# junyanz/interactive-deep-colorization

Hardware: NVIDIA B200
Metric: net_forward images/sec @256x256 (higher is better)
Workload: dtype f16x2-split operands, f32 accumulate (ab within 1e-3 of the f32 reference)

## Files before the change

### interactive_deep_colorization_b200/csrc/idc_api.cu

```cuda
#include <math.h>
#include <stdarg.h>
#include <stdio.h>
#include <string.h>

#include <algorithm>

#include "idc_internal.h"

using namespace idc;

struct idc_ctx : public idc::Ctx {};

namespace {

int fail(Ctx* c, int code, const char* fmt, ...) {
  char buf[512];
  va_list ap;
  va_start(ap, fmt);
  vsnprintf(buf, sizeof(buf), fmt, ap);
  va_end(ap);
  if (c) c->err = buf;
  return code;
}

// ... 616 lines not shown
  c->simt = flags & IDC_FLAG_ENGINE_SIMT;
  c->fast = (flags & IDC_FLAG_FAST_FP16) && !c->simt;
  c->dist = flags & IDC_FLAG_DIST;
  c->glob = flags & IDC_FLAG_GLOBAL_HINTS;
  c->caffe313 = flags & IDC_FLAG_CAFFE313;
  build_plan(c);
  int rc = alloc_workspace(c);
  if (rc != IDC_OK) {
    fprintf(stderr, "idc_create: %s\n", c->err.c_str());
    idc_destroy(c);
    return rc;
  }
  cudaStreamCreateWithFlags(&c->own_stream, cudaStreamNonBlocking);
  *out = c;
  return IDC_OK;
}

int idc_set_option(idc_ctx* c, const char* name, int value) {
  if (!c || !name) return IDC_ERR_ARG;
  struct { const char* n; int* v; } tab[] = {
      {"halo", &c->opt.halo}, {"pairs", &c->opt.pairs}, {"mt", &c->opt.mt}, {"chunk_kb", &c->opt.chunk_kb},
      {"split_k", &c->opt.split_k}, {"direct_stores", &c->opt.direct_stores}, {"host_pipe", &c->opt.host_pipe},
      {"pdl", &c->opt.pdl}, {"split_pairs", &c->opt.split_pairs}, {"tanh_scale", &c->opt.tanh_scale},
      {"side_dist", &c->opt.side_dist}, {"split_bn128", &c->opt.split_bn128}, {"halo_split", &c->opt.halo_split}, {"prologue_sync2", &c->opt.prologue_sync2}, {"chain", &c->opt.chain}, {"conv1_1_umma", &c->opt.conv1_1_umma}};
  for (auto& t : tab)
    if (!strcmp(t.n, name)) {
      *t.v = value;
      if (c->weights_ready && strcmp(name, "host_pipe") && strcmp(name, "tanh_scale") && strcmp(name, "side_dist") && strcmp(name, "conv1_1_umma")) {
        CUDA_TRY(c, cudaSetDevice(c->dev));
        CUDA_TRY(c, cudaDeviceSynchronize());
        int rc = plan_engines(c);
        if (rc != IDC_OK) return rc;
      }
      if (c->graph_exec) { cudaGraphExecDestroy(c->graph_exec); c->graph_exec = nullptr; }
      return IDC_OK;
    }
  return fail(c, IDC_ERR_KEY, "unknown option '%s'", name);
}

int idc_load_tensor(idc_ctx* c, const char* key, const void* data, int dtype, int ndim, const int64_t* dims) {
  if (!c || !key || !data || ndim < 0 || ndim > 8 || (ndim && !dims)) return fail(c, IDC_ERR_ARG, "bad load_tensor args");
  HostTensor t;
  size_t count = 1;
  for (int i = 0; i < ndim; ++i) {
    if (dims[i] < 0) return fail(c, IDC_ERR_ARG, "negative dim");
    t.dims.push_back(dims[i]);
    count *= (size_t)dims[i];
// ... 728 lines not shown
```

### interactive_deep_colorization_b200/csrc/idc_internal.h

```cpp
#pragma once
#include <cuda.h>
#include <cuda_fp16.h>
#include <cuda_runtime.h>
#include <stdint.h>

#include <map>
#include <string>
#include <vector>

#include "../../include/idc_b200.h"

namespace idc {

constexpr int kMaxTaps = 34;
constexpr int kMaxSrc = 6;
constexpr int kMaxCls = 4;

enum Act { ACT_NONE = 0, ACT_RELU = 1, ACT_LEAKY02 = 2 };

constexpr int kActScaleLog2 = 6;
constexpr float kActScale = 64.0f;
constexpr float kActInvScale = 1.0f / 64.0f;

struct Tap {
// ... 55 lines not shown
  double flops_per_image = 0;
};

struct Conv11Weights {
  float w[36 * 64];
  float b[64];
};

struct Options {
  int halo = 1;
  int pairs = 1;
  int mt = -1;
  int chunk_kb = -1;
  int split_k = -1;
  int direct_stores = 0;
  int host_pipe = 1;
  int pdl = 1;
  int split_pairs = 1;
  int split_bn128 = 1;
  int conv1_1_umma = 1;
  int chain = 0;
  int prologue_sync2 = 1;
  int halo_split = 0;
  int side_dist = 1;
  int tanh_scale = 110;
};

struct HostTensor {
  std::vector<float> data;
  std::vector<int64_t> dims;
};

struct Ctx {
  int dev = 0;
  int max_n = 0, H = 0, W = 0;
  unsigned flags = 0;
  Options opt;
  bool simt = false, fast = false, dist = false, glob = false;
  std::map<std::string, HostTensor> raw;
  std::vector<ActBuf> bufs;
  std::map<std::string, int> buf_index;
  std::vector<ConvOp> ops;
  char* arena = nullptr;
  size_t arena_bytes = 0;
  bool weights_ready = false;
  float* w11 = nullptr;
// ... 122 lines not shown
```

### interactive_deep_colorization_b200/csrc/idc_umma.cu

```cuda
#include <stdio.h>
#include <stdlib.h>

#include "idc_internal.h"

#ifndef IDC_CTA_COUNTERS
#define IDC_CTA_COUNTERS 0
#endif

namespace idc {

constexpr int kBM = 128;
constexpr int kBK = 64;
constexpr int kThreads = 384;
constexpr int kCtrlRegs = 56;
constexpr int kAccRegs = 224;
constexpr int kAccThreads = 256;

struct UmmaParams {
  const CUtensorMap* amaps;
  const int4* kblk;
  int nkb, ncls;
  int chunk_kb;
  int split_k;
  float* ws;
// ... 2 lines not shown
  int hbox, wbox, wshift;
  int Hl, Wl, cout_pad;
  const float* bias;
  const float* scale;
  const float* shift;
  const float* gadd;
  int gadd_ld;
  float gadd_mult;
  int act;
  __half* out_hi;
  __half* out_lo;
  int Hout, Wout, Cout, os;
  int store_mode;
  float* out_f32;
  int out_ld;
  const float* wout;
  const float* bout;
  float* out_ab;
  float out_mult;
  int* err;
  long long* dbgbuf;
  int n_amaps;
  int max_ctas;
  int halo_groups;
  int prologue_sync2;
  int img0;
};

__device__ __forceinline__ uint32_t smem_u32(const void* p) { return (uint32_t)__cvta_generic_to_shared(p); }

__device__ __forceinline__ void mbar_init(uint32_t bar, uint32_t count) {
  asm volatile("mbarrier.init.shared::cta.b64 [%0], %1;" ::"r"(bar), "r"(count));
}
__device__ __forceinline__ void mbar_expect_tx(uint32_t bar, uint32_t bytes) {
  asm volatile("mbarrier.arrive.expect_tx.shared::cta.b64 _, [%0], %1;" ::"r"(bar), "r"(bytes) : "memory");
}
__device__ __forceinline__ void mbar_arrive(uint32_t bar) {
  asm volatile("mbarrier.arrive.shared::cta.b64 _, [%0];" ::"r"(bar) : "memory");
}
__device__ __forceinline__ uint32_t mbar_try_wait(uint32_t bar, uint32_t parity) {
  uint32_t ok;
  asm volatile(
      "{\n\t.reg .pred p;\n\t"
      "mbarrier.try_wait.parity.shared::cta.b64 p, [%1], %2;\n\t"
      "selp.u32 %0, 1, 0, p;\n\t}"
      : "=r"(ok)
      : "r"(bar), "r"(parity)
// ... 168 lines not shown
  return r;
}

template <bool SPLIT>
__device__ __forceinline__ void split_pack(const float (&f)[32], uint32_t (&hw)[16], uint32_t (&lw)[16]) {
#pragma unroll
  for (int j = 0; j < 16; ++j) {
    hw[j] = pack_f16x2_sat(f[2 * j], f[2 * j + 1]);
    if (SPLIT) {
      const float2 hf = __half22float2(*reinterpret_cast<const __half2*>(&hw[j]));
      lw[j] = pack_f16x2_sat(f[2 * j] - hf.x, f[2 * j + 1] - hf.y);
    }
  }
}

__device__ __forceinline__ void split_h(float v, __half& hi, __half& lo) {
  v = fminf(fmaxf(v, -65504.f), 65504.f);
  hi = __float2half_rn(v);
  lo = __float2half_rn(v - __half2float(hi));
}

constexpr int kHaloW = 10, kHaloH = 18;
constexpr int kHaloPlane = (kHaloW * kHaloH * 128 + 1023) / 1024 * 1024;
template <int BN, int MT, int CG, bool SPLIT, bool HALO = false>
struct SmemPlan {
  static constexpr int kABytes = MT * kBM * kBK * 2;
  static constexpr int kAStage = HALO ? 0 : kABytes;
  static constexpr int kBBytes = (BN / CG) * kBK * 2;
  static constexpr int kStageBytes = (SPLIT ? 2 : 1) * (kAStage + kBBytes);
  static constexpr int kHaloSlot = (SPLIT ? 2 : 1) * kHaloPlane;
  static constexpr int kHaloBytes = HALO ? 2 * kHaloSlot : 0;
  static_assert(!HALO || MT == 1, "halo tiles are single 16x8-pixel M-tiles");
  static constexpr int kTail = 3 * BN * 4 + 272 * 4 + 256 + 128 * 2 * 4;
  static constexpr int kOutStage = 16384;
  static constexpr int kBudget = 232448 - 1024 - kTail - kOutStage - kHaloBytes;
  static constexpr int kStages = kBudget / kStageBytes >= 4 ? 4 : kBudget / kStageBytes;
  static constexpr int kTotal = kStages * kStageBytes + kHaloBytes + kOutStage + kTail + 1024;
  static constexpr int kBufCols = MT * BN;
  static constexpr int kNBuf = (512 / kBufCols) >= 4 ? 4 : (512 / kBufCols);
  static constexpr int kTmemCols = (kNBuf * kBufCols <= 128) ? 128 : (kNBuf * kBufCols <= 256 ? 256 : 512);
  static constexpr int kCH = (MT == 2) ? BN : BN / 2;
  static_assert(kStages >= 2, "need at least a double-buffered operand ring");
  static_assert(CG == 1 || BN == 256 || BN == 128 || BN == 64, "pairs: BN/2 weight rows per CTA must be a whole number of swizzle atoms");
};

template <int BN, int MT, int CG, bool SPLIT, bool HALO, bool CHAIN>
__device__ __forceinline__ void conv_body(const CUtensorMap* bhi_list, const CUtensorMap* blo_list,
                                          const UmmaParams* plist, const int nl, int* gridbar) {
  static_assert(!(HALO && CHAIN), "chained launches use per-tap boxes");
  using SP = SmemPlan<BN, MT, CG, SPLIT, HALO>;
  const UmmaParams& p0 = plist[0];
  constexpr int STAGES = SP::kStages;
  constexpr bool PAIR = CG == 2;
  extern __shared__ uint8_t smem_raw[];
  uint8_t* smem = reinterpret_cast<uint8_t*>((reinterpret_cast<uintptr_t>(smem_raw) + 1023) & ~uintptr_t(1023));
  uint8_t* s_halo = smem + STAGES * SP::kStageBytes;
  uint8_t* s_out = s_halo + SP::kHaloBytes;
  uint8_t* tail = s_out + SP::kOutStage;
  float* s_bias = reinterpret_cast<float*>(tail);
  float* s_scale = s_bias + BN;
  float* s_shift = s_scale + BN;
  float* s_head = s_shift + BN;
  uint64_t* s_bar = reinterpret_cast<uint64_t*>(s_head + 272);
  constexpr int NBUF = SP::kNBuf;
  uint64_t* full_bar = s_bar;
  uint64_t* empty_bar = s_bar + STAGES;
  uint64_t* tfull_bar = s_bar + 2 * STAGES;
  uint64_t* tempty_bar = s_bar + 2 * STAGES + NBUF;
  uint32_t* s_tmem = reinterpret_cast<uint32_t*>(s_bar + 2 * STAGES + 2 * NBUF);
  uint64_t* afull_bar = s_bar + 20;
  uint64_t* aempty_bar = s_bar + 22;
  float* s_red = reinterpret_cast<float*>(s_bar + 32);

  const int warp = threadIdx.x >> 5, lane = threadIdx.x & 31;
  const long long t_kernel0 = (IDC_CTA_COUNTERS && p0.dbgbuf) ? clock64() : 0;

  if (!CHAIN && p0.wout) {
    for (int i = threadIdx.x; i < 256; i += kThreads) s_head[i] = p0.wout[i];
    if (threadIdx.x < 2) s_head[256 + threadIdx.x] = p0.bout[threadIdx.x];
  }
  const uint32_t cta_rank = PAIR ? cluster_ctarank() : 0u;
  const bool leader = cta_rank == 0;
  if (threadIdx.x == 32) {
    prefetch_tmap(bhi_list);
    if (SPLIT) prefetch_tmap(blo_list);
    for (int i = 0; i < p0.n_amaps; ++i) prefetch_tmap(p0.amaps + i);
  }
  if (threadIdx.x == 0) {
    for (int s = 0; s < STAGES; ++s) {
      mbar_init(smem_u32(&full_bar[s]), CG);
      mbar_init(smem_u32(&empty_bar[s]), 1);
    }
    for (int a = 0; a < NBUF; ++a) {
      mbar_init(smem_u32(&tfull_bar[a]), 1);
      mbar_init(smem_u32(&tempty_bar[a]), 8 * CG);
    }
    if (HALO)
      for (int a = 0; a < 2; ++a) {
        mbar_init(smem_u32(&afull_bar[a]), CG);
        mbar_init(smem_u32(&aempty_bar[a]), 1);
      }
    asm volatile("fence.mbarrier_init.release.cluster;" ::: "memory");
  }
  if (PAIR && p0.prologue_sync2) cluster_sync_all();
  if (warp == 1) {
    if (PAIR) {
      asm volatile("tcgen05.alloc.cta_group::2.sync.aligned.shared::cta.b32 [%0], %1;" ::"r"(smem_u32(s_tmem)),
                   "r"((uint32_t)SP::kTmemCols)
                   : "memory");
      asm volatile("tcgen05.relinquish_alloc_permit.cta_group::2.sync.aligned;" ::: "memory");
    } else {
      asm volatile("tcgen05.alloc.cta_group::1.sync.aligned.shared::cta.b32 [%0], %1;" ::"r"(smem_u32(s_tmem)),
                   "r"((uint32_t)SP::kTmemCols)
                   : "memory");
      asm volatile("tcgen05.relinquish_alloc_permit.cta_group::1.sync.aligned;" ::: "memory");
    }
  }
  tc_fence_before();
  if (PAIR) cluster_sync_all(); else __syncthreads();
  tc_fence_after();
  const uint32_t tmem_base = *s_tmem;
// ... 58 lines not shown
        pdl_wait();
      } else if (w0 < p.total_tiles * S) {
        grid_wait(gridbar, l * (int)gridDim.x, p.err);
        asm volatile("fence.proxy.async;" ::: "memory");
      }
      for (int w = w0; w < p.total_tiles * S; w += gridDim.x / CG) {
        const int tile = w / S, ks = w - tile * S;
        const int kbeg = (ks * p.nkb) / S, kend = ((ks + 1) * p.nkb) / S;
        const int kpre = (w == w0) ? kbeg + npre : kbeg;
        int r = tile;
        const int nt = r % p.n_tiles_n;
        r /= p.n_tiles_n;
        const int cls = r % p.ncls;
        r /= p.ncls;
        if (PAIR) r = 2 * r + (int)cta_rank;
        const int img_rel = r / tiles_per_img;
        r -= img_rel * tiles_per_img;
        const int img = p.img0 + img_rel;
        const int y0 = (r / p.tiles_x) * (p.hbox * MT), x0 = (r % p.tiles_x) * p.wbox;
        const int brow = cls * p.cout_pad + nt * BN + (int)cta_rank * (BN / CG);
        const int4* kb = p.kblk + cls * p.nkb;
        if (HALO) {
          for (int k = kbeg; k < kend; ++k) {
            if (k % 9 == 0) {
              const uint32_t slot = hcount & 1, hphase = (hcount >> 1) & 1;
              ++hcount;
              mbar_wait(smem_u32(&aempty_bar[slot]), hphase ^ 1, p.err, 6);
              if (elect_one()) {
                const uint32_t fa = smem_u32(&afull_bar[slot]);
                const uint32_t sh = smem_u32(s_halo + slot * SP::kHaloSlot);
                const int c0 = (k / 9) * kBK;
                constexpr uint32_t kHaloTx = (SPLIT ? 2 : 1) * kHaloW * kHaloH * 128;
                if (PAIR) {
                  if (leader) mbar_expect_tx(fa, 2 * kHaloTx); else mbar_arrive_rank0(fa);
                  tma_load_4d_pair(sh, p.amaps, fa, c0, x0 - 1, y0 - 1, img);
                  if (SPLIT) tma_load_4d_pair(sh + kHaloPlane, p.amaps + 1, fa, c0, x0 - 1, y0 - 1, img);
                } else {
                  mbar_expect_tx(fa, kHaloTx);
                  tma_load_4d(sh, p.amaps, fa, c0, x0 - 1, y0 - 1, img);
                  if (SPLIT) tma_load_4d(sh + kHaloPlane, p.amaps + 1, fa, c0, x0 - 1, y0 - 1, img);
                }
              }
              __syncwarp();
            }
            mbar_wait(smem_u32(&empty_bar[stage]), phase ^ 1, p.err, 1);
            if (k >= kpre && elect_one()) {
              const uint32_t fb = smem_u32(&full_bar[stage]);
              const int4 e = __ldg(kb + k);
              const uint32_t sb = smem_u32(smem + stage * SP::kStageBytes);
              if (PAIR) {
                if (leader) mbar_expect_tx(fb, 2 * SP::kStageBytes); else mbar_arrive_rank0(fb);
                tma_load_2d_pair(sb, &bmap_hi, fb, e.y, brow);
                if (SPLIT) tma_load_2d_pair(sb + SP::kBBytes, &bmap_lo, fb, e.y, brow);
              } else {
                mbar_expect_tx(fb, SP::kStageBytes);
                tma_load_2d(sb, &bmap_hi, fb, e.y, brow);
                if (SPLIT) tma_load_2d(sb + SP::kBBytes, &bmap_lo, fb, e.y, brow);
              }
            }
            __syncwarp();
            if (++stage == STAGES) { stage = 0; phase ^= 1; }
          }
        }
        if (!HALO)
        for (int k = kbeg; k < kend; ++k) {
          mbar_wait(smem_u32(&empty_bar[stage]), phase ^ 1, p.err, 1);
          if (elect_one()) {
            const uint32_t fb = smem_u32(&full_bar[stage]);
            const int4 e = __ldg(kb + k);
            const uint32_t sa = smem_u32(smem + stage * SP::kStageBytes);
            const CUtensorMap* am = p.amaps + e.x;
// ... 19 lines not shown
          }
          __syncwarp();
          if (++stage == STAGES) { stage = 0; phase ^= 1; }
        }
      }
      }
    }
  } else if (warp == 1 && leader) {
    {
      constexpr uint32_t idesc = make_idesc(BN, kBM * CG);
      int stage = 0;
      uint32_t phase = 0;
      uint32_t cc = 0;
      uint32_t hcount = 0;
      long long t_wait_tempty = 0, t_wait_full = 0, t_first_full = 0;
      const long long t_start = clock64();
      for (int l = 0; l < n_layers; ++l) {
      const UmmaParams& p = plist[l];
      const int G = p.chunk_kb;
      const int S = p.split_k;
      for (int w = blockIdx.x / CG; w < p.total_tiles * S; w += gridDim.x / CG) {
        const int ks = w % S;
        const int kbeg = (ks * p.nkb) / S, kend = ((ks + 1) * p.nkb) / S;
        for (int k0 = kbeg; k0 < kend; k0 += G, ++cc) {
          const uint32_t buf = cc % NBUF;
          const uint32_t bphase = (cc / NBUF) & 1;
          const long long tA = (IDC_CTA_COUNTERS && p.dbgbuf) ? clock64() : 0;
          mbar_wait(smem_u32(&tempty_bar[buf]), bphase ^ 1, p.err, 2);
          if (IDC_CTA_COUNTERS && p.dbgbuf) t_wait_tempty += clock64() - tA;
          tc_fence_after();
          const uint32_t d_tmem = tmem_base + buf * SP::kBufCols;
          const int k1 = (k0 + G < kend) ? k0 + G : kend;
          for (int k = k0; k < k1; ++k) {
            const long long tB = (IDC_CTA_COUNTERS && p.dbgbuf) ? clock64() : 0;
            uint32_t hslot = 0;
            if (HALO) {
              if (k % 9 == 0) {
                mbar_wait(smem_u32(&afull_bar[hcount & 1]), (hcount >> 1) & 1, p.err, 7);
                ++hcount;
              }
              hslot = (hcount - 1) & 1;
            }
            mbar_wait(smem_u32(&full_bar[stage]), phase, p.err, 3);
            if (IDC_CTA_COUNTERS && p.dbgbuf) {
              t_wait_full += clock64() - tB;
              if (t_first_full == 0) t_first_full = clock64() - t_kernel0;
            }
            tc_fence_after();
            if (elect_one()) {
            const uint32_t sa = smem_u32(smem + stage * SP::kStageBytes);
            const uint32_t sb = sa + (SPLIT ? 2 : 1) * SP::kAStage;
            const uint64_t b_hi = make_sw128_desc(sb);
            const uint64_t b_lo = make_sw128_desc(sb + SP::kBBytes);
            const uint32_t fresh = (k == k0) ? 0u : 1u;
            uint32_t ha = 0;
            if (HALO) {
              const int4 e = __ldg(p.kblk + k);
              ha = smem_u32(s_halo + hslot * SP::kHaloSlot) + (uint32_t)(e.z * kHaloW + e.w) * 128u;
            }
#pragma unroll
            for (int mt = 0; mt < MT; ++mt) {
              const uint64_t a_hi = HALO ? make_sw128_desc(ha, kHaloW * 128) : make_sw128_desc(sa + mt * (kBM * kBK * 2));
              const uint64_t a_lo = HALO ? make_sw128_desc(ha + kHaloPlane, kHaloW * 128)
                                         : make_sw128_desc(sa + SP::kABytes + mt * (kBM * kBK * 2));
              const uint32_t d = d_tmem + mt * BN;
              uint32_t first = fresh;
              if (SPLIT) {
#pragma unroll
                for (int kk = 0; kk < kBK / 16; ++kk) {
                  const uint64_t adv = (uint64_t)(kk * 2);
                  if (PAIR) {
                    umma_f16_pair(d, a_lo + adv, b_hi + adv, idesc, first);
                    umma_f16_pair(d, a_hi + adv, b_lo + adv, idesc, 1u);
                  } else {
                    umma_f16(d, a_lo + adv, b_hi + adv, idesc, first);
                    umma_f16(d, a_hi + adv, b_lo + adv, idesc, 1u);
                  }
                  first = 1u;
                }
              }
#pragma unroll
              for (int kk = 0; kk < kBK / 16; ++kk) {
                const uint64_t adv = (uint64_t)(kk * 2);
                if (PAIR) umma_f16_pair(d, a_hi + adv, b_hi + adv, idesc, first);
                else umma_f16(d, a_hi + adv, b_hi + adv, idesc, first);
                first = 1u;
              }
            }
            if (PAIR) {
              umma_commit_pair(smem_u32(&empty_bar[stage]));
              if (HALO && k % 9 == 8) umma_commit_pair(smem_u32(&aempty_bar[hslot]));
              if (k == k1 - 1) umma_commit_pair(smem_u32(&tfull_bar[buf]));
            } else {
              umma_commit(smem_u32(&empty_bar[stage]));
              if (HALO && k % 9 == 8) umma_commit(smem_u32(&aempty_bar[hslot]));
              if (k == k1 - 1) umma_commit(smem_u32(&tfull_bar[buf]));
            }
            }
            __syncwarp();
            if (++stage == STAGES) { stage = 0; phase ^= 1; }
          }
        }
      }
      }
      if (IDC_CTA_COUNTERS && p0.dbgbuf && lane == 0) {
        const UmmaParams& p = p0;
        p.dbgbuf[blockIdx.x * 16 + 0] = clock64() - t_start;
        p.dbgbuf[blockIdx.x * 16 + 1] = t_wait_tempty;
        p.dbgbuf[blockIdx.x * 16 + 2] = t_wait_full;
        p.dbgbuf[blockIdx.x * 16 + 6] = t_first_full;
        p.dbgbuf[blockIdx.x * 16 + 10] = t_start - t_kernel0;
      }
    }
  } else if (warp >= 4) {
    asm volatile("setmaxnreg.inc.sync.aligned.u32 %0;" ::"n"(kAccRegs));
    constexpr int CH = SP::kCH;
    const int quarter = warp & 3;
    const int half = (warp - 4) >> 2;
// ... 302 lines not shown

  if (IDC_CTA_COUNTERS && p0.dbgbuf && warp == 4 && lane == 0) {
    const UmmaParams& p = p0;
    p.dbgbuf[blockIdx.x * 16 + 3] = t_wait_tfull_g;
    p.dbgbuf[blockIdx.x * 16 + 4] = t_drain_g;
    p.dbgbuf[blockIdx.x * 16 + 5] = t_epi_g;
    p.dbgbuf[blockIdx.x * 16 + 7] = clock64() - t_kernel0;
    p.dbgbuf[blockIdx.x * 16 + 8] = t_splitk_g;
    p.dbgbuf[blockIdx.x * 16 + 9] = t_spin_g;
  }
  tc_fence_before();
  if (PAIR) cluster_sync_all(); else __syncthreads();
  if (warp == 1) {
    __syncwarp();
    if (PAIR)
      asm volatile("tcgen05.dealloc.cta_group::2.sync.aligned.b32 %0, %1;" ::"r"(tmem_base), "r"((uint32_t)SP::kTmemCols)
                   : "memory");
    else
      asm volatile("tcgen05.dealloc.cta_group::1.sync.aligned.b32 %0, %1;" ::"r"(tmem_base), "r"((uint32_t)SP::kTmemCols)
                   : "memory");
  }
}

template <int BN, int MT, int CG, bool SPLIT, bool HALO = false>
__global__ void __launch_bounds__(kThreads, 1)
umma_conv_kernel(const __grid_constant__ CUtensorMap bmap_hi, const __grid_constant__ CUtensorMap bmap_lo,
                 const __grid_constant__ UmmaParams p) {
  conv_body<BN, MT, CG, SPLIT, HALO, false>(&bmap_hi, &bmap_lo, &p, 1, nullptr);
}

constexpr int kChainMax = 20;
struct ChainParams {
  CUtensorMap bhi[kChainMax], blo[kChainMax];
  UmmaParams layer[kChainMax];
  int nl;
  int* gridbar;
};
template <int BN, int MT, int CG, bool SPLIT>
__global__ void __launch_bounds__(kThreads, 1) umma_chain_kernel(const __grid_constant__ ChainParams P) {
  conv_body<BN, MT, CG, SPLIT, false, true>(P.bhi, P.blo, P.layer, P.nl, P.gridbar);
}

constexpr int kC11K = 48;
constexpr int kC11PackBytes = 2 * 8192 + 2 * 64 * 4;
constexpr int kC11Smem = 2 * 16384 + kC11PackBytes + 64 + 1024;

__device__ __forceinline__ uint32_t sw128_off(int row, int chunk) {
  return (uint32_t)((row >> 3) * 1024 + (row & 7) * 128 + ((chunk ^ (row & 7)) << 4));
}

__global__ void conv1_1_pack_kernel(const float* __restrict__ w36x64, const float* __restrict__ bias, uint8_t* __restrict__ out) {
  const int co = threadIdx.x;
  if (co >= 64) return;
  float mx = 0.f;
  for (int k = 0; k < 36; ++k) mx = fmaxf(mx, fabsf(w36x64[k * 64 + co]));
  int e = 0;
  if (mx > 0.f) { int ex; frexpf(mx, &ex); e = 9 - ex; }
  const float sc = ldexpf(1.f, e);
  __half* bh = reinterpret_cast<__half*>(out);
  __half* bl = reinterpret_cast<__half*>(out + 8192);
  for (int k = 0; k < 64; ++k) {
    const float v = k < 36 ? w36x64[k * 64 + co] * sc : 0.f;
    __half hi, lo;
// ... 210 lines not shown
static PFN_encodeTiled get_encode() {
  static PFN_encodeTiled fn = nullptr;
  if (!fn) {
    void* p = nullptr;
    cudaDriverEntryPointQueryResult q;
    if (cudaGetDriverEntryPoint("cuTensorMapEncodeTiled", &p, cudaEnableDefault, &q) == cudaSuccess &&
        q == cudaDriverEntryPointSuccess)
      fn = (PFN_encodeTiled)p;
  }
  return fn;
}

struct UmmaPlan {
  CUtensorMap* d_amaps = nullptr;
  int4* d_kblk = nullptr;
  CUtensorMap bmap_hi, bmap_lo;
  UmmaParams prm{};
  int num_sms = 148;
  int dev = 0;
  int mt = 1;
  int cg = 1;
  int split_k = 1;
  bool halo = false;
  size_t ws_floats = 0;
  int ws_tiles = 0;
};

struct ViewKey {
  int src, s, qy, qx;
  bool operator==(const ViewKey& o) const { return src == o.src && s == o.s && qy == o.qy && qx == o.qx; }
};

static int floordiv2(int v) { return v >= 0 ? v / 2 : -((-v + 1) / 2); }

template <int BN, int MT, int CG, bool SPLIT, bool HALO = false>
static cudaError_t launch_inst(const UmmaPlan& pl, const UmmaParams& prm, cudaStream_t st, bool pdl) {
  using SP = SmemPlan<BN, MT, CG, SPLIT, HALO>;
  static unsigned long long attr_devs = 0;
  if (pl.dev >= 64 || !(attr_devs & (1ull << pl.dev))) {
    cudaError_t e = cudaFuncSetAttribute(umma_conv_kernel<BN, MT, CG, SPLIT, HALO>, cudaFuncAttributeMaxDynamicSharedMemorySize,
                                         SP::kTotal);
    if (e != cudaSuccess) return e;
    if (pl.dev < 64) attr_devs |= 1ull << pl.dev;
  }
  const long items = (long)prm.total_tiles * prm.split_k;
  int grid = items * CG < pl.num_sms ? (int)items * CG : (pl.num_sms / CG) * CG;
  if (prm.max_ctas > 0 && grid > prm.max_ctas) grid = prm.max_ctas;
  cudaLaunchConfig_t cfg{};
  cfg.gridDim = dim3(grid);
  cfg.blockDim = dim3(kThreads);
  cfg.dynamicSmemBytes = SP::kTotal;
  cfg.stream = st;
  cudaLaunchAttribute at[2];
  int na = 0;
  if (CG > 1) {
    at[na].id = cudaLaunchAttributeClusterDimension;
    at[na].val.clusterDim.x = CG; at[na].val.clusterDim.y = 1; at[na].val.clusterDim.z = 1;
    ++na;
  }
  if (pdl) {
    at[na].id = cudaLaunchAttributeProgrammaticStreamSerialization;
    at[na].val.programmaticStreamSerializationAllowed = 1;
    ++na;
  }
  cfg.attrs = at;
  cfg.numAttrs = na;
  return cudaLaunchKernelEx(&cfg, umma_conv_kernel<BN, MT, CG, SPLIT, HALO>, pl.bmap_hi, pl.bmap_lo, prm);
}

int umma_plan_op(Ctx* c, ConvOp& op) {
  PFN_encodeTiled enc = get_encode();
  if (!enc) { c->err = "cuTensorMapEncodeTiled entry point not available"; return IDC_ERR_CUDA; }
  umma_free_op(op);
  UmmaPlan* pl = new UmmaPlan();
  op.umma_plan = pl;
  cudaDeviceProp prop;
  cudaGetDeviceProperties(&prop, c->dev);
  pl->num_sms = prop.multiProcessorCount;
  pl->dev = c->dev;
  op.bn_tile = (op.cout_pad % 256 == 0) ? 256 : (op.cout_pad % 192 == 0) ? 192 : (op.cout_pad % 128 == 0) ? 128 : 64;
  if (op.cout_pad % op.bn_tile) { c->err = "cout not tileable: " + op.name; return IDC_ERR_ARG; }
  int best = 1 << 30;
  for (int wb = 128; wb >= 8; wb >>= 1) {
    const int hb = kBM / wb;
    const int t = ceil_div(op.Wl, wb) * ceil_div(op.Hl, hb);
    if (t < best) { best = t; op.wbox = wb; op.hbox = hb; }
  }
  bool halo_shape = false;
  {
    const int mode = c->opt.halo;
    bool ok = mode >= 1 && !c->fast && op.ncls == 1 && op.ntaps == 9;
    unsigned seen = 0;
    for (int t = 0; ok && t < op.ntaps; ++t) {
      const Tap& tp = op.taps[0][t];
      if (tp.src != op.taps[0][0].src || op.src[tp.src].s != 1 || tp.ty < -1 || tp.ty > 1 || tp.tx < -1 || tp.tx > 1) ok = false;
      else seen |= 1u << ((tp.ty + 1) * 3 + tp.tx + 1);
    }
    if (ok && (seen != 0x1FFu || op.src[op.taps[0][0].src].cin % kBK)) ok = false;
    halo_shape = ok;
    if (ok && !(op.bn_tile == 128 || (mode >= 3 && op.bn_tile == 64))) ok = false;
    if (ok) {
      const long T = (long)c->max_n * ceil_div(op.Hl, 16) * ceil_div(op.Wl, 8) * (op.cout_pad / op.bn_tile);
      if (T < 2L * pl->num_sms && mode < 3) ok = false;
    }
    pl->halo = ok;
    if (ok) { op.wbox = 8; op.hbox = 16; }
  }
  pl->mt = 1;
  if (op.bn_tile <= 128 && !pl->halo) {
    const long tiles2 = (long)op.ncls * c->max_n * ceil_div(op.Hl, 2 * op.hbox) * ceil_div(op.Wl, op.wbox) *
                        (op.cout_pad / op.bn_tile);
    if (tiles2 >= 2L * pl->num_sms && op.hbox * 2 <= 256) pl->mt = 2;
  }
  { const int v = c->opt.mt; if (!pl->halo && (v == 1 || (v == 2 && op.bn_tile <= 128))) pl->mt = v; }
  pl->cg = 1;
  {
    const long tiles1 = (long)op.ncls * c->max_n * ceil_div(op.Hl, op.hbox) * ceil_div(op.Wl, op.wbox) * (op.cout_pad / op.bn_tile);
    const bool can = !c->fast && (op.bn_tile == 256 || op.bn_tile == 128 || (op.bn_tile == 64 && (pl->mt == 2 || pl->halo)));
    const long tiles_mt = tiles1 / pl->mt;
    const int mode = c->opt.pairs;
    if (can && (mode >= 2 || (mode == 1 && tiles_mt >= 2L * pl->num_sms))) pl->cg = 2;
  }
  const int nkb = op.K / kBK;
  {
    const int ty = ceil_div(op.Hl, op.hbox * pl->mt), tx = ceil_div(op.Wl, op.wbox), ntn = op.cout_pad / op.bn_tile;
    const long m_tiles = (long)c->max_n * ty * tx;
    const long T = (long)op.ncls * m_tiles * ntn;
    int S = 1;
    const bool eligible = nkb >= 8 && !op.fuse_out_head && pl->mt == 1 && pl->cg == 1 && !pl->halo;
    if (T * 2 <= pl->num_sms && eligible) {
      S = (int)(pl->num_sms / T);
      if (S > nkb / 4) S = nkb / 4;
      if (S > op.bn_tile / 32) S = op.bn_tile / 32;
      if (S < 1) S = 1;
    }
    {
      const int v = c->opt.split_k;
      if (v >= 1 && v <= nkb && v <= op.bn_tile / 32 && pl->mt == 1 && !pl->halo && pl->cg == 1 && T * v <= pl->num_sms) S = v;
    }
    long Tw = T;
    if (S > 1 && c->opt.split_pairs && !c->fast && (op.bn_tile == 256 || op.bn_tile == 128)) {
      const long T2 = (long)op.ncls * ((m_tiles + 1) / 2) * ntn;
      int S2 = (int)((pl->num_sms / 2) / T2);
      if (S2 > nkb / 4) S2 = nkb / 4;
      if (S2 > op.bn_tile / 32) S2 = op.bn_tile / 32;
// ... 3 lines not shown
        const int ntn2 = op.cout_pad / 128;
        const long T3 = (long)op.ncls * ((m_tiles + 1) / 2) * ntn2;
        int S3 = (int)((pl->num_sms / 2) / T3);
        if (S3 > nkb / 4) S3 = nkb / 4;
        if (S3 > 4) S3 = 4;
        if (c->opt.split_k >= 1 && c->opt.split_k <= S3) S3 = c->opt.split_k;
        if (S3 >= 2) { op.bn_tile = 128; S = S3; Tw = T3 * 2; }
        if (S3 >= 2 && c->opt.halo_split && halo_shape && nkb % 9 == 0 && (nkb / 9) % S3 == 0 &&
            ceil_div(op.Hl, 16) * ceil_div(op.Wl, 8) == ty * tx) {
          pl->halo = true;
          op.wbox = 8; op.hbox = 16;
        }
      }
    }
    pl->split_k = S;
    pl->ws_tiles = (int)Tw;
    pl->ws_floats = S > 1 ? (size_t)Tw * S * kBM * op.bn_tile : 0;
    if (pl->ws_floats > c->splitk_ws_floats) c->splitk_ws_floats = pl->ws_floats;
    if (S > 1 && pl->ws_tiles > c->splitk_max_tiles) c->splitk_max_tiles = pl->ws_tiles;
  }
  std::vector<ViewKey> views;
  std::vector<int4> kblk((size_t)op.ncls * nkb);
  if (pl->halo) {
    const int src = op.taps[0][0].src, groups = op.src[src].cin / kBK;
    views.push_back(ViewKey{src, 1, 0, 0});
    for (int i = 0; i < nkb; ++i) {
      const int g = i / 9, t = i % 9;
      kblk[i] = make_int4(0, (t * groups + g) * kBK, op.taps[0][t].ty + 1, op.taps[0][t].tx + 1);
    }
  }
  for (int cls = 0; cls < op.ncls && !pl->halo; ++cls) {
    int kb = 0;
    for (int t = 0; t < op.ntaps; ++t) {
      const Tap& tp = op.taps[cls][t];
      const int s = op.src[tp.src].s;
      ViewKey vk{tp.src, s, 0, 0};
      int dy = tp.ty, dx = tp.tx;
      if (s == 2) {
        vk.qy = ((tp.ty % 2) + 2) % 2; vk.qx = ((tp.tx % 2) + 2) % 2;
        dy = floordiv2(tp.ty); dx = floordiv2(tp.tx);
      }
      int vi = -1;
      for (size_t i = 0; i < views.size(); ++i)
        if (views[i] == vk) vi = (int)i;
      if (vi < 0) { views.push_back(vk); vi = (int)views.size() - 1; }
      const int cin = op.src[tp.src].cin;
      if (cin % kBK) { c->err = "cin not a multiple of 64: " + op.name; return IDC_ERR_ARG; }
      for (int c0 = 0; c0 < cin; c0 += kBK) kblk[(size_t)cls * nkb + kb++] = make_int4(vi * 2, c0, dy, dx);
    }
    if (kb != nkb) { c->err = "k-block count mismatch: " + op.name; return IDC_ERR_ARG; }
  }
  std::vector<CUtensorMap> amaps(views.size() * 2);
  for (size_t i = 0; i < views.size(); ++i) {
    const ViewKey& vk = views[i];
    const ActBuf& b = c->bufs[op.src[vk.src].buf];
    const int Hv = (b.H - vk.qy + vk.s - 1) / vk.s, Wv = (b.W - vk.qx + vk.s - 1) / vk.s;
    for (int part = 0; part < 2; ++part) {
      char* base = (char*)(part == 0 ? b.p0 : b.p1);
      if (!base) { amaps[i * 2 + part] = amaps[i * 2]; continue; }
      base += ((size_t)vk.qy * b.W + vk.qx) * b.C * sizeof(__half);
      cuuint64_t dims[4] = {(cuuint64_t)b.C, (cuuint64_t)Wv, (cuuint64_t)Hv, (cuuint64_t)c->max_n};
      cuuint64_t strides[3] = {(cuuint64_t)vk.s * b.C * 2, (cuuint64_t)vk.s * b.W * b.C * 2,
                               (cuuint64_t)b.H * b.W * b.C * 2};
      cuuint32_t box[4] = {(cuuint32_t)kBK, (cuuint32_t)(pl->halo ? kHaloW : op.wbox),
                           (cuuint32_t)(pl->halo ? kHaloH : op.hbox * pl->mt), 1};
      cuuint32_t estr[4] = {1, 1, 1, 1};
      CUresult r = enc(&amaps[i * 2 + part], CU_TENSOR_MAP_DATA_TYPE_FLOAT16, 4, base, dims, strides, box, estr,
                       CU_TENSOR_MAP_INTERLEAVE_NONE, CU_TENSOR_MAP_SWIZZLE_128B, CU_TENSOR_MAP_L2_PROMOTION_L2_128B,
// ... 12 lines not shown
    cuuint32_t box[2] = {(cuuint32_t)kBK, (cuuint32_t)(op.bn_tile / pl->cg)};
    cuuint32_t estr[2] = {1, 1};
    CUresult r = enc(part == 0 ? &pl->bmap_hi : &pl->bmap_lo, CU_TENSOR_MAP_DATA_TYPE_FLOAT16, 2,
                     part == 0 ? (void*)op.w_hi : (void*)op.w_lo, dims, strides, box, estr,
                     CU_TENSOR_MAP_INTERLEAVE_NONE, CU_TENSOR_MAP_SWIZZLE_128B, CU_TENSOR_MAP_L2_PROMOTION_L2_256B,
                     CU_TENSOR_MAP_FLOAT_OOB_FILL_NONE);
    if (r != CUDA_SUCCESS) {
      char msg[256];
      snprintf(msg, sizeof(msg), "cuTensorMapEncodeTiled(B) failed (%d) for op %s", (int)r, op.name.c_str());
      c->err = msg;
      return IDC_ERR_CUDA;
    }
  }
  if (cudaMalloc(&pl->d_amaps, amaps.size() * sizeof(CUtensorMap)) != cudaSuccess ||
      cudaMalloc(&pl->d_kblk, kblk.size() * sizeof(int4)) != cudaSuccess) {
    c->err = "cudaMalloc failed in umma_plan_op";
    return IDC_ERR_CUDA;
  }
  cudaMemcpy(pl->d_amaps, amaps.data(), amaps.size() * sizeof(CUtensorMap), cudaMemcpyHostToDevice);
  cudaMemcpy(pl->d_kblk, kblk.data(), kblk.size() * sizeof(int4), cudaMemcpyHostToDevice);

  UmmaParams& q = pl->prm;
  q.amaps = pl->d_amaps; q.n_amaps = (int)amaps.size(); q.kblk = pl->d_kblk; q.nkb = nkb; q.ncls = op.ncls;
  q.halo_groups = pl->halo ? nkb / 9 : 0;
  {
    const int natural = (op.cout_pad % 256 == 0) ? 256 : (op.cout_pad % 192 == 0) ? 192 : (op.cout_pad % 128 == 0) ? 128 : 64;
    int g = c->fast ? 4 : (natural <= 128 ? 2 : 1);
    if (c->opt.chunk_kb >= 1) g = c->opt.chunk_kb;
    q.chunk_kb = g;
  }
  q.tiles_y = ceil_div(op.Hl, op.hbox * pl->mt); q.tiles_x = ceil_div(op.Wl, op.wbox);
  q.n_tiles_n = op.cout_pad / op.bn_tile;
  q.hbox = op.hbox; q.wbox = op.wbox;
  q.wshift = 0;
  while ((1 << q.wshift) < op.wbox) q.wshift++;
  q.Hl = op.Hl; q.Wl = op.Wl; q.cout_pad = op.cout_pad;
  q.bias = op.epi.bias; q.scale = op.epi.scale; q.shift = op.epi.shift;
  q.gadd = nullptr; q.gadd_ld = 512; q.gadd_mult = kActScale;
  q.act = op.epi.act;
  if (op.out_f32) {
    q.out_f32 = op.out_f32_ptr; q.out_ld = op.cout_pad;
  } else if (op.out_buf >= 0) {
    const ActBuf& ob = c->bufs[op.out_buf];
    q.out_hi = (__half*)ob.p0; q.out_lo = (__half*)ob.p1;
    q.Hout = ob.H; q.Wout = ob.W; q.Cout = ob.C; q.os = op.os;
  }
  if (op.fuse_out_head) { q.wout = c->wout; q.bout = c->bout; }
// ... 49 lines not shown
         !op.fuse_out_head && !op.out_f32 && op.out_buf >= 0;
}

cudaError_t umma_run_chain(Ctx* c, int first, int last, int n, cudaStream_t st) {
  const int nl = last - first + 1;
  if (nl < 2 || nl > kChainMax || !c->chain_bar) return cudaErrorInvalidValue;
  ChainParams P;
  int grid = 0, dev = 0;
  for (int k = 0; k < nl; ++k) {
    ConvOp& op = c->ops[first + k];
    if (!umma_op_chainable(c, op)) return cudaErrorInvalidValue;
    UmmaPlan* pl = static_cast<UmmaPlan*>(op.umma_plan);
    cudaError_t e = umma_prepare(c, op, n, nullptr, (float)c->opt.tanh_scale, 0, 0, P.layer[k]);
    if (e != cudaSuccess) return e;
    P.layer[k].dbgbuf = nullptr;
    P.bhi[k] = pl->bmap_hi; P.blo[k] = pl->bmap_lo;
    const long items = (long)P.layer[k].total_tiles * P.layer[k].split_k;
    if (items * 2 > pl->num_sms) return cudaErrorInvalidValue;
    if (items * 2 > grid) grid = (int)items * 2;
    dev = pl->dev;
  }
  P.nl = nl;
  P.gridbar = c->chain_bar;
  using SP = SmemPlan<128, 1, 2, true, false>;
  static unsigned long long attr_devs = 0;
  if (dev >= 64 || !(attr_devs & (1ull << dev))) {
    cudaError_t e = cudaFuncSetAttribute(umma_chain_kernel<128, 1, 2, true>, cudaFuncAttributeMaxDynamicSharedMemorySize, SP::kTotal);
    if (e != cudaSuccess) return e;
    if (dev < 64) attr_devs |= 1ull << dev;
  }
  cudaLaunchConfig_t cfg{};
  cfg.gridDim = dim3(grid);
  cfg.blockDim = dim3(kThreads);
  cfg.dynamicSmemBytes = SP::kTotal;
  cfg.stream = st;
  cudaLaunchAttribute at[2];
  int na = 0;
  at[na].id = cudaLaunchAttributeClusterDimension;
  at[na].val.clusterDim.x = 2; at[na].val.clusterDim.y = 1; at[na].val.clusterDim.z = 1;
  ++na;
  if (pdl_take(c)) {
    at[na].id = cudaLaunchAttributeProgrammaticStreamSerialization;
    at[na].val.programmaticStreamSerializationAllowed = 1;
    ++na;
  }
  cfg.attrs = at;
  cfg.numAttrs = na;
  c->launch_count++;
  return cudaLaunchKernelEx(&cfg, umma_chain_kernel<128, 1, 2, true>, P);
}

cudaError_t umma_run_op(Ctx* c, ConvOp& op, int n, float* out_ab_fused, float out_mult, cudaStream_t st, int img0,
                        int max_ctas) {
  UmmaPlan* pl = static_cast<UmmaPlan*>(op.umma_plan);
  if (!pl) return cudaErrorInvalidValue;
  UmmaParams prm;
  cudaError_t pe = umma_prepare(c, op, n, out_ab_fused, out_mult, img0, max_ctas, prm);
  if (pe != cudaSuccess) return pe;
  c->launch_count++;
  const bool split = !c->fast;
  const bool pdl = pdl_take(c);
#define IDC_LAUNCH(BN_, MT_, CG_)                                              \
  return split ? launch_inst<BN_, MT_, CG_, true>(*pl, prm, st, pdl) : launch_inst<BN_, MT_, CG_, false>(*pl, prm, st, pdl)
  if (pl->halo) {
    if (!split) return cudaErrorInvalidValue;
    switch (op.bn_tile * 10 + pl->cg) {
      case 641: return launch_inst<64, 1, 1, true, true>(*pl, prm, st, pdl);
      case 642: return launch_inst<64, 1, 2, true, true>(*pl, prm, st, pdl);
      case 1281: return launch_inst<128, 1, 1, true, true>(*pl, prm, st, pdl);
      case 1282: return launch_inst<128, 1, 2, true, true>(*pl, prm, st, pdl);
      default: return cudaErrorInvalidValue;
    }
  }
  switch (op.bn_tile * 100 + pl->mt * 10 + pl->cg) {
    case 6411: IDC_LAUNCH(64, 1, 1);
    case 6421: IDC_LAUNCH(64, 2, 1);
    case 12811: IDC_LAUNCH(128, 1, 1);
    case 12821: IDC_LAUNCH(128, 2, 1);
    case 19211: IDC_LAUNCH(192, 1, 1);
    case 25611: IDC_LAUNCH(256, 1, 1);
    case 25612: IDC_LAUNCH(256, 1, 2);
    case 12812: IDC_LAUNCH(128, 1, 2);
    case 12822: IDC_LAUNCH(128, 2, 2);
    case 6422: IDC_LAUNCH(64, 2, 2);
    default: return cudaErrorInvalidValue;
  }
#undef IDC_LAUNCH
}

}
```

Measured before the change: 2773.

## Extend halo-tile A staging to strided convs and upsample ops with tagged groups

Generalizes the halo path, which loads one 10x18 pixel tile per channel group and reuses it across taps. It now also covers stride-2 convolutions and transposed/upsample ops whose taps map into a 3x3 neighbourhood of a parity view. A host-built k-block table tags where each halo group opens and closes and which view map it uses, replacing the fixed k%9 grouping. It also adds an optional third halo ring slot for 128-wide paired tiles. The aim is to cut per-tap A-operand TMA traffic on these layers, at the cost of more shared memory per CTA and uneven group lengths that the interleaved long/short ordering tries to smooth.

```diff
diff --git a/interactive_deep_colorization_b200/csrc/idc_api.cu b/interactive_deep_colorization_b200/csrc/idc_api.cu
--- a/interactive_deep_colorization_b200/csrc/idc_api.cu
+++ b/interactive_deep_colorization_b200/csrc/idc_api.cu
@@ -662,7 +662,7 @@
       {"halo", &c->opt.halo}, {"pairs", &c->opt.pairs}, {"mt", &c->opt.mt}, {"chunk_kb", &c->opt.chunk_kb},
       {"split_k", &c->opt.split_k}, {"direct_stores", &c->opt.direct_stores}, {"host_pipe", &c->opt.host_pipe},
       {"pdl", &c->opt.pdl}, {"split_pairs", &c->opt.split_pairs}, {"tanh_scale", &c->opt.tanh_scale},
-      {"side_dist", &c->opt.side_dist}, {"split_bn128", &c->opt.split_bn128}, {"halo_split", &c->opt.halo_split}, {"prologue_sync2", &c->opt.prologue_sync2}, {"chain", &c->opt.chain}, {"conv1_1_umma", &c->opt.conv1_1_umma}};
+      {"side_dist", &c->opt.side_dist}, {"split_bn128", &c->opt.split_bn128}, {"halo_split", &c->opt.halo_split}, {"halo_up", &c->opt.halo_up}, {"halo_slots", &c->opt.halo_slots}, {"prologue_sync2", &c->opt.prologue_sync2}, {"chain", &c->opt.chain}, {"conv1_1_umma", &c->opt.conv1_1_umma}};
   for (auto& t : tab)
     if (!strcmp(t.n, name)) {
       *t.v = value;
diff --git a/interactive_deep_colorization_b200/csrc/idc_internal.h b/interactive_deep_colorization_b200/csrc/idc_internal.h
--- a/interactive_deep_colorization_b200/csrc/idc_internal.h
+++ b/interactive_deep_colorization_b200/csrc/idc_internal.h
@@ -101,6 +101,8 @@
   int chain = 0;
   int prologue_sync2 = 1;
   int halo_split = 0;
+  int halo_up = 1;
+  int halo_slots = 2;
   int side_dist = 1;
   int tanh_scale = 110;
 };
diff --git a/interactive_deep_colorization_b200/csrc/idc_umma.cu b/interactive_deep_colorization_b200/csrc/idc_umma.cu
--- a/interactive_deep_colorization_b200/csrc/idc_umma.cu
+++ b/interactive_deep_colorization_b200/csrc/idc_umma.cu
@@ -48,7 +48,6 @@
   long long* dbgbuf;
   int n_amaps;
   int max_ctas;
-  int halo_groups;
   int prologue_sync2;
   int img0;
 };
@@ -263,15 +262,23 @@
 
 constexpr int kHaloW = 10, kHaloH = 18;
 constexpr int kHaloPlane = (kHaloW * kHaloH * 128 + 1023) / 1024 * 1024;
-template <int BN, int MT, int CG, bool SPLIT, bool HALO = false>
+constexpr int kHaloOpen = 1, kHaloClose = 2;
+__host__ __device__ constexpr int halo_tag(bool open, bool close, int amap, int c0) {
+  return (open ? kHaloOpen : 0) | (close ? kHaloClose : 0) | (amap << 2) | (c0 << 10);
+}
+__device__ __forceinline__ int halo_tag_amap(int x) { return (x >> 2) & 255; }
+__device__ __forceinline__ int halo_tag_c0(int x) { return x >> 10; }
+template <int BN, int MT, int CG, bool SPLIT, int HS = 0>
 struct SmemPlan {
+  static constexpr bool HALO = HS > 0;
   static constexpr int kABytes = MT * kBM * kBK * 2;
   static constexpr int kAStage = HALO ? 0 : kABytes;
   static constexpr int kBBytes = (BN / CG) * kBK * 2;
   static constexpr int kStageBytes = (SPLIT ? 2 : 1) * (kAStage + kBBytes);
   static constexpr int kHaloSlot = (SPLIT ? 2 : 1) * kHaloPlane;
-  static constexpr int kHaloBytes = HALO ? 2 * kHaloSlot : 0;
+  static constexpr int kHaloBytes = HS * kHaloSlot;
   static_assert(!HALO || MT == 1, "halo tiles are single 16x8-pixel M-tiles");
+  static_assert(HS == 0 || HS == 2 || HS == 3, "halo ring: 2 or 3 slots");
   static constexpr int kTail = 3 * BN * 4 + 272 * 4 + 256 + 128 * 2 * 4;
   static constexpr int kOutStage = 16384;
   static constexpr int kBudget = 232448 - 1024 - kTail - kOutStage - kHaloBytes;
@@ -282,14 +289,16 @@
   static constexpr int kTmemCols = (kNBuf * kBufCols <= 128) ? 128 : (kNBuf * kBufCols <= 256 ? 256 : 512);
   static constexpr int kCH = (MT == 2) ? BN : BN / 2;
   static_assert(kStages >= 2, "need at least a double-buffered operand ring");
+  static_assert(HS < 3 || kStages == 4, "a third halo slot must not cost weight stages");
   static_assert(CG == 1 || BN == 256 || BN == 128 || BN == 64, "pairs: BN/2 weight rows per CTA must be a whole number of swizzle atoms");
 };
 
-template <int BN, int MT, int CG, bool SPLIT, bool HALO, bool CHAIN>
+template <int BN, int MT, int CG, bool SPLIT, int HS, bool CHAIN>
 __device__ __forceinline__ void conv_body(const CUtensorMap* bhi_list, const CUtensorMap* blo_list,
                                           const UmmaParams* plist, const int nl, int* gridbar) {
+  constexpr bool HALO = HS > 0;
   static_assert(!(HALO && CHAIN), "chained launches use per-tap boxes");
-  using SP = SmemPlan<BN, MT, CG, SPLIT, HALO>;
+  using SP = SmemPlan<BN, MT, CG, SPLIT, HS>;
   const UmmaParams& p0 = plist[0];
   constexpr int STAGES = SP::kStages;
   constexpr bool PAIR = CG == 2;
@@ -310,7 +319,7 @@
   uint64_t* tempty_bar = s_bar + 2 * STAGES + NBUF;
   uint32_t* s_tmem = reinterpret_cast<uint32_t*>(s_bar + 2 * STAGES + 2 * NBUF);
   uint64_t* afull_bar = s_bar + 20;
-  uint64_t* aempty_bar = s_bar + 22;
+  uint64_t* aempty_bar = s_bar + 20 + HS;
   float* s_red = reinterpret_cast<float*>(s_bar + 32);
 
   const int warp = threadIdx.x >> 5, lane = threadIdx.x & 31;
@@ -337,7 +346,7 @@
       mbar_init(smem_u32(&tempty_bar[a]), 8 * CG);
     }
     if (HALO)
-      for (int a = 0; a < 2; ++a) {
+      for (int a = 0; a < HS; ++a) {
         mbar_init(smem_u32(&afull_bar[a]), CG);
         mbar_init(smem_u32(&aempty_bar[a]), 1);
       }
@@ -442,23 +451,25 @@
         const int4* kb = p.kblk + cls * p.nkb;
         if (HALO) {
           for (int k = kbeg; k < kend; ++k) {
-            if (k % 9 == 0) {
-              const uint32_t slot = hcount & 1, hphase = (hcount >> 1) & 1;
+            const int4 e = __ldg(kb + k);
+            if (e.x & kHaloOpen) {
+              const uint32_t slot = hcount % HS, hphase = (hcount / HS) & 1;
               ++hcount;
               mbar_wait(smem_u32(&aempty_bar[slot]), hphase ^ 1, p.err, 6);
               if (elect_one()) {
                 const uint32_t fa = smem_u32(&afull_bar[slot]);
                 const uint32_t sh = smem_u32(s_halo + slot * SP::kHaloSlot);
-                const int c0 = (k / 9) * kBK;
+                const CUtensorMap* am = p.amaps + halo_tag_amap(e.x);
+                const int c0 = halo_tag_c0(e.x);
                 constexpr uint32_t kHaloTx = (SPLIT ? 2 : 1) * kHaloW * kHaloH * 128;
                 if (PAIR) {
                   if (leader) mbar_expect_tx(fa, 2 * kHaloTx); else mbar_arrive_rank0(fa);
-                  tma_load_4d_pair(sh, p.amaps, fa, c0, x0 - 1, y0 - 1, img);
-                  if (SPLIT) tma_load_4d_pair(sh + kHaloPlane, p.amaps + 1, fa, c0, x0 - 1, y0 - 1, img);
+                  tma_load_4d_pair(sh, am, fa, c0, x0 - 1, y0 - 1, img);
+                  if (SPLIT) tma_load_4d_pair(sh + kHaloPlane, am + 1, fa, c0, x0 - 1, y0 - 1, img);
                 } else {
                   mbar_expect_tx(fa, kHaloTx);
-                  tma_load_4d(sh, p.amaps, fa, c0, x0 - 1, y0 - 1, img);
-                  if (SPLIT) tma_load_4d(sh + kHaloPlane, p.amaps + 1, fa, c0, x0 - 1, y0 - 1, img);
+                  tma_load_4d(sh, am, fa, c0, x0 - 1, y0 - 1, img);
+                  if (SPLIT) tma_load_4d(sh + kHaloPlane, am + 1, fa, c0, x0 - 1, y0 - 1, img);
                 }
               }
               __syncwarp();
@@ -466,7 +477,6 @@
             mbar_wait(smem_u32(&empty_bar[stage]), phase ^ 1, p.err, 1);
             if (k >= kpre && elect_one()) {
               const uint32_t fb = smem_u32(&full_bar[stage]);
-              const int4 e = __ldg(kb + k);
               const uint32_t sb = smem_u32(smem + stage * SP::kStageBytes);
               if (PAIR) {
                 if (leader) mbar_expect_tx(fb, 2 * SP::kStageBytes); else mbar_arrive_rank0(fb);
@@ -532,6 +542,8 @@
       for (int w = blockIdx.x / CG; w < p.total_tiles * S; w += gridDim.x / CG) {
         const int ks = w % S;
         const int kbeg = (ks * p.nkb) / S, kend = ((ks + 1) * p.nkb) / S;
+        const int cls = (w / S / p.n_tiles_n) % p.ncls;
+        const int4* kb = p.kblk + cls * p.nkb;
         for (int k0 = kbeg; k0 < kend; k0 += G, ++cc) {
           const uint32_t buf = cc % NBUF;
           const uint32_t bphase = (cc / NBUF) & 1;
@@ -544,12 +556,14 @@
           for (int k = k0; k < k1; ++k) {
             const long long tB = (IDC_CTA_COUNTERS && p.dbgbuf) ? clock64() : 0;
             uint32_t hslot = 0;
+            int4 e = make_int4(0, 0, 0, 0);
             if (HALO) {
-              if (k % 9 == 0) {
-                mbar_wait(smem_u32(&afull_bar[hcount & 1]), (hcount >> 1) & 1, p.err, 7);
+              e = __ldg(kb + k);
+              if (e.x & kHaloOpen) {
+                mbar_wait(smem_u32(&afull_bar[hcount % HS]), (hcount / HS) & 1, p.err, 7);
                 ++hcount;
               }
-              hslot = (hcount - 1) & 1;
+              hslot = (hcount - 1) % HS;
             }
             mbar_wait(smem_u32(&full_bar[stage]), phase, p.err, 3);
             if (IDC_CTA_COUNTERS && p.dbgbuf) {
@@ -564,10 +578,7 @@
             const uint64_t b_lo = make_sw128_desc(sb + SP::kBBytes);
             const uint32_t fresh = (k == k0) ? 0u : 1u;
             uint32_t ha = 0;
-            if (HALO) {
-              const int4 e = __ldg(p.kblk + k);
-              ha = smem_u32(s_halo + hslot * SP::kHaloSlot) + (uint32_t)(e.z * kHaloW + e.w) * 128u;
-            }
+            if (HALO) ha = smem_u32(s_halo + hslot * SP::kHaloSlot) + (uint32_t)(e.z * kHaloW + e.w) * 128u;
 #pragma unroll
             for (int mt = 0; mt < MT; ++mt) {
               const uint64_t a_hi = HALO ? make_sw128_desc(ha, kHaloW * 128) : make_sw128_desc(sa + mt * (kBM * kBK * 2));
@@ -599,11 +610,11 @@
             }
             if (PAIR) {
               umma_commit_pair(smem_u32(&empty_bar[stage]));
-              if (HALO && k % 9 == 8) umma_commit_pair(smem_u32(&aempty_bar[hslot]));
+              if (HALO && (e.x & kHaloClose)) umma_commit_pair(smem_u32(&aempty_bar[hslot]));
               if (k == k1 - 1) umma_commit_pair(smem_u32(&tfull_bar[buf]));
             } else {
               umma_commit(smem_u32(&empty_bar[stage]));
-              if (HALO && k % 9 == 8) umma_commit(smem_u32(&aempty_bar[hslot]));
+              if (HALO && (e.x & kHaloClose)) umma_commit(smem_u32(&aempty_bar[hslot]));
               if (k == k1 - 1) umma_commit(smem_u32(&tfull_bar[buf]));
             }
             }
@@ -952,11 +963,11 @@
   }
 }
 
-template <int BN, int MT, int CG, bool SPLIT, bool HALO = false>
+template <int BN, int MT, int CG, bool SPLIT, int HS = 0>
 __global__ void __launch_bounds__(kThreads, 1)
 umma_conv_kernel(const __grid_constant__ CUtensorMap bmap_hi, const __grid_constant__ CUtensorMap bmap_lo,
                  const __grid_constant__ UmmaParams p) {
-  conv_body<BN, MT, CG, SPLIT, HALO, false>(&bmap_hi, &bmap_lo, &p, 1, nullptr);
+  conv_body<BN, MT, CG, SPLIT, HS, false>(&bmap_hi, &bmap_lo, &p, 1, nullptr);
 }
 
 constexpr int kChainMax = 20;
@@ -968,7 +979,7 @@
 };
 template <int BN, int MT, int CG, bool SPLIT>
 __global__ void __launch_bounds__(kThreads, 1) umma_chain_kernel(const __grid_constant__ ChainParams P) {
-  conv_body<BN, MT, CG, SPLIT, false, true>(P.bhi, P.blo, P.layer, P.nl, P.gridbar);
+  conv_body<BN, MT, CG, SPLIT, 0, true>(P.bhi, P.blo, P.layer, P.nl, P.gridbar);
 }
 
 constexpr int kC11K = 48;
@@ -1225,6 +1236,7 @@
   int cg = 1;
   int split_k = 1;
   bool halo = false;
+  int halo_slots = 2;
   size_t ws_floats = 0;
   int ws_tiles = 0;
 };
@@ -1236,12 +1248,74 @@
 
 static int floordiv2(int v) { return v >= 0 ? v / 2 : -((-v + 1) / 2); }
 
-template <int BN, int MT, int CG, bool SPLIT, bool HALO = false>
+static ViewKey tap_view(const ConvOp& op, const Tap& tp, int& dy, int& dx) {
+  const int s = op.src[tp.src].s;
+  ViewKey vk{tp.src, s, 0, 0};
+  dy = tp.ty; dx = tp.tx;
+  if (s == 2) {
+    vk.qy = ((tp.ty % 2) + 2) % 2; vk.qx = ((tp.tx % 2) + 2) % 2;
+    dy = floordiv2(tp.ty); dx = floordiv2(tp.tx);
+  }
+  return vk;
+}
+
+static int view_index(std::vector<ViewKey>& views, const ViewKey& vk) {
+  for (size_t i = 0; i < views.size(); ++i)
+    if (views[i] == vk) return (int)i;
+  views.push_back(vk);
+  return (int)views.size() - 1;
+}
+
+static bool halo_up_shape(const ConvOp& op) {
+  const bool strided_conv = op.kind == OP_CONV && op.nsrc == 1 && op.ncls == 1 && op.ntaps == 9 && op.src[0].s == 2;
+  if (!strided_conv && op.kind != OP_UP) return false;
+  for (int s = 0; s < op.nsrc; ++s)
+    if (op.src[s].cin % kBK) return false;
+  for (int cls = 0; cls < op.ncls; ++cls)
+    for (int t = 0; t < op.ntaps; ++t) {
+      int dy, dx;
+      tap_view(op, op.taps[cls][t], dy, dx);
+      if (dy < -1 || dy > 1 || dx < -1 || dx > 1) return false;
+    }
+  return true;
+}
+
+static void halo_table(const ConvOp& op, int cls, std::vector<ViewKey>& views, int4* out) {
+  struct Group { int view, c0; std::vector<int4> kb; };
+  std::vector<Group> groups;
+  int kcol = 0;
+  for (int t = 0; t < op.ntaps; ++t) {
+    const Tap& tp = op.taps[cls][t];
+    int dy, dx;
+    const int vi = view_index(views, tap_view(op, tp, dy, dx));
+    for (int c0 = 0; c0 < op.src[tp.src].cin; c0 += kBK, kcol += kBK) {
+      size_t g = 0;
+      while (g < groups.size() && !(groups[g].view == vi && groups[g].c0 == c0)) ++g;
+      if (g == groups.size()) groups.push_back(Group{vi, c0, {}});
+      groups[g].kb.push_back(make_int4(0, kcol, dy + 1, dx + 1));
+    }
+  }
+  std::vector<const Group*> lng, shrt, order;
+  for (const Group& g : groups) (g.kb.size() >= 4 ? lng : shrt).push_back(&g);
+  for (size_t i = 0; i < lng.size() || i < shrt.size(); ++i) {
+    if (i < lng.size()) order.push_back(lng[i]);
+    if (i < shrt.size()) order.push_back(shrt[i]);
+  }
+  int k = 0;
+  for (const Group* g : order)
+    for (size_t j = 0; j < g->kb.size(); ++j) {
+      int4 e = g->kb[j];
+      e.x = halo_tag(j == 0, j + 1 == g->kb.size(), g->view * 2, g->c0);
+      out[k++] = e;
+    }
+}
+
+template <int BN, int MT, int CG, bool SPLIT, int HS = 0>
 static cudaError_t launch_inst(const UmmaPlan& pl, const UmmaParams& prm, cudaStream_t st, bool pdl) {
-  using SP = SmemPlan<BN, MT, CG, SPLIT, HALO>;
+  using SP = SmemPlan<BN, MT, CG, SPLIT, HS>;
   static unsigned long long attr_devs = 0;
   if (pl.dev >= 64 || !(attr_devs & (1ull << pl.dev))) {
-    cudaError_t e = cudaFuncSetAttribute(umma_conv_kernel<BN, MT, CG, SPLIT, HALO>, cudaFuncAttributeMaxDynamicSharedMemorySize,
+    cudaError_t e = cudaFuncSetAttribute(umma_conv_kernel<BN, MT, CG, SPLIT, HS>, cudaFuncAttributeMaxDynamicSharedMemorySize,
                                          SP::kTotal);
     if (e != cudaSuccess) return e;
     if (pl.dev < 64) attr_devs |= 1ull << pl.dev;
@@ -1268,7 +1342,7 @@
   }
   cfg.attrs = at;
   cfg.numAttrs = na;
-  return cudaLaunchKernelEx(&cfg, umma_conv_kernel<BN, MT, CG, SPLIT, HALO>, pl.bmap_hi, pl.bmap_lo, prm);
+  return cudaLaunchKernelEx(&cfg, umma_conv_kernel<BN, MT, CG, SPLIT, HS>, pl.bmap_hi, pl.bmap_lo, prm);
 }
 
 int umma_plan_op(Ctx* c, ConvOp& op) {
@@ -1290,6 +1364,7 @@
     if (t < best) { best = t; op.wbox = wb; op.hbox = hb; }
   }
   bool halo_shape = false;
+  bool halo_up_op = false;
   {
     const int mode = c->opt.halo;
     bool ok = mode >= 1 && !c->fast && op.ncls == 1 && op.ntaps == 9;
@@ -1301,12 +1376,14 @@
     }
     if (ok && (seen != 0x1FFu || op.src[op.taps[0][0].src].cin % kBK)) ok = false;
     halo_shape = ok;
+    if (!ok && mode >= 1 && !c->fast && c->opt.halo_up && halo_up_shape(op)) ok = halo_up_op = true;
     if (ok && !(op.bn_tile == 128 || (mode >= 3 && op.bn_tile == 64))) ok = false;
     if (ok) {
       const long T = (long)c->max_n * ceil_div(op.Hl, 16) * ceil_div(op.Wl, 8) * (op.cout_pad / op.bn_tile);
       if (T < 2L * pl->num_sms && mode < 3) ok = false;
     }
     pl->halo = ok;
+    if (!ok) halo_up_op = false;
     if (ok) { op.wbox = 8; op.hbox = 16; }
   }
   pl->mt = 1;
@@ -1324,6 +1401,7 @@
     const int mode = c->opt.pairs;
     if (can && (mode >= 2 || (mode == 1 && tiles_mt >= 2L * pl->num_sms))) pl->cg = 2;
   }
+  if (halo_up_op && c->opt.halo_slots == 3 && op.bn_tile == 128 && pl->cg == 2) pl->halo_slots = 3;
   const int nkb = op.K / kBK;
   {
     const int ty = ceil_div(op.Hl, op.hbox * pl->mt), tx = ceil_div(op.Wl, op.wbox), ntn = op.cout_pad / op.bn_tile;
@@ -1373,28 +1451,14 @@
   std::vector<ViewKey> views;
   std::vector<int4> kblk((size_t)op.ncls * nkb);
   if (pl->halo) {
-    const int src = op.taps[0][0].src, groups = op.src[src].cin / kBK;
-    views.push_back(ViewKey{src, 1, 0, 0});
-    for (int i = 0; i < nkb; ++i) {
-      const int g = i / 9, t = i % 9;
-      kblk[i] = make_int4(0, (t * groups + g) * kBK, op.taps[0][t].ty + 1, op.taps[0][t].tx + 1);
-    }
+    for (int cls = 0; cls < op.ncls; ++cls) halo_table(op, cls, views, kblk.data() + (size_t)cls * nkb);
   }
   for (int cls = 0; cls < op.ncls && !pl->halo; ++cls) {
     int kb = 0;
     for (int t = 0; t < op.ntaps; ++t) {
       const Tap& tp = op.taps[cls][t];
-      const int s = op.src[tp.src].s;
-      ViewKey vk{tp.src, s, 0, 0};
-      int dy = tp.ty, dx = tp.tx;
-      if (s == 2) {
-        vk.qy = ((tp.ty % 2) + 2) % 2; vk.qx = ((tp.tx % 2) + 2) % 2;
-        dy = floordiv2(tp.ty); dx = floordiv2(tp.tx);
-      }
-      int vi = -1;
-      for (size_t i = 0; i < views.size(); ++i)
-        if (views[i] == vk) vi = (int)i;
-      if (vi < 0) { views.push_back(vk); vi = (int)views.size() - 1; }
+      int dy, dx;
+      const int vi = view_index(views, tap_view(op, tp, dy, dx));
       const int cin = op.src[tp.src].cin;
       if (cin % kBK) { c->err = "cin not a multiple of 64: " + op.name; return IDC_ERR_ARG; }
       for (int c0 = 0; c0 < cin; c0 += kBK) kblk[(size_t)cls * nkb + kb++] = make_int4(vi * 2, c0, dy, dx);
@@ -1453,7 +1517,6 @@
 
   UmmaParams& q = pl->prm;
   q.amaps = pl->d_amaps; q.n_amaps = (int)amaps.size(); q.kblk = pl->d_kblk; q.nkb = nkb; q.ncls = op.ncls;
-  q.halo_groups = pl->halo ? nkb / 9 : 0;
   {
     const int natural = (op.cout_pad % 256 == 0) ? 256 : (op.cout_pad % 192 == 0) ? 192 : (op.cout_pad % 128 == 0) ? 128 : 64;
     int g = c->fast ? 4 : (natural <= 128 ? 2 : 1);
@@ -1549,7 +1612,7 @@
   }
   P.nl = nl;
   P.gridbar = c->chain_bar;
-  using SP = SmemPlan<128, 1, 2, true, false>;
+  using SP = SmemPlan<128, 1, 2, true, 0>;
   static unsigned long long attr_devs = 0;
   if (dev >= 64 || !(attr_devs & (1ull << dev))) {
     cudaError_t e = cudaFuncSetAttribute(umma_chain_kernel<128, 1, 2, true>, cudaFuncAttributeMaxDynamicSharedMemorySize, SP::kTotal);
@@ -1591,11 +1654,12 @@
   return split ? launch_inst<BN_, MT_, CG_, true>(*pl, prm, st, pdl) : launch_inst<BN_, MT_, CG_, false>(*pl, prm, st, pdl)
   if (pl->halo) {
     if (!split) return cudaErrorInvalidValue;
-    switch (op.bn_tile * 10 + pl->cg) {
-      case 641: return launch_inst<64, 1, 1, true, true>(*pl, prm, st, pdl);
-      case 642: return launch_inst<64, 1, 2, true, true>(*pl, prm, st, pdl);
-      case 1281: return launch_inst<128, 1, 1, true, true>(*pl, prm, st, pdl);
-      case 1282: return launch_inst<128, 1, 2, true, true>(*pl, prm, st, pdl);
+    switch (op.bn_tile * 100 + pl->cg * 10 + pl->halo_slots) {
+      case 6412: return launch_inst<64, 1, 1, true, 2>(*pl, prm, st, pdl);
+      case 6422: return launch_inst<64, 1, 2, true, 2>(*pl, prm, st, pdl);
+      case 12812: return launch_inst<128, 1, 1, true, 2>(*pl, prm, st, pdl);
+      case 12822: return launch_inst<128, 1, 2, true, 2>(*pl, prm, st, pdl);
+      case 12823: return launch_inst<128, 1, 2, true, 3>(*pl, prm, st, pdl);
       default: return cudaErrorInvalidValue;
     }
   }
```

Result: faster. 2827, median of 6 (+1.9%).
